# ssheybani/baby-vision-curriculum

Measured on AMD Instinct MI355X. Metric: video clips/sec (node) VideoMAE-base 16x224^2 bf16 pretraining, higher is better.
Workload: dtype bf16; 1 GPU; VideoMAE-base (ViT-B/16 encoder, 4-layer decoder), 16x224x224 clips, tubelet 2, 90% tube mask, full training step (fwd + MSE + bwd + GradScaler + SGD-Nesterov); clips_per_gpu=256, global_batch=256, parallelism=dp1, weights=random init N(0,0.02), seed 0

## Files before the change

baby-vision-curriculum_amd/csrc/attention.hip:

```cpp
#include <stdlib.h>

#include "attention.h"

namespace bvc {

#define AS3 __attribute__((address_space(3)))
#define MFMA32(a, b, c) __builtin_amdgcn_mfma_f32_32x32x16_bf16((a), (b), (c), 0, 0, 0)

template <int HD>
__device__ __forceinline__ int swz_dual(int r) {
    if constexpr (HD == 64) return (((r >> 1) & 1) << 2) | ((r >> 2) & 3);
    else return (r >> 2) & 3;
}

template <int HD>
constexpr int pan_w(int p) { return HD - 64 * p >= 64 ? 64 : HD - 64 * p; }
constexpr int img_hd(int hd) { return hd == 80 || hd == 88 ? 96 : hd; }
constexpr uint32_t kDmaZero = 0xfffffff0u;
__device__ __forceinline__ int swz_pw(int pw, int r) { return pw == 64 ? swz_dual<64>(r) : swz_dual<32>(r); }

template <int PW, int NW, int VC = PW / 8>
__device__ __forceinline__ void stage_panel(__amdgpu_buffer_rsrc_t rs, int row0, int ld, int col0, char* lds, int GB, int wave, int lane) {
    constexpr int CPR = PW / 8;
    constexpr int RPP = 64 / CPR;
#pragma unroll
    for (int jj = 0; jj < (PW / 8 + NW - 1) / NW; ++jj) {
        const int j = wave + NW * jj;
        if (NW > PW / 8 && j >= PW / 8) break;
        const int r = RPP * j + lane / CPR;
        const int c = (lane % CPR) ^ swz_dual<PW>(r);
        uint32_t off = (uint32_t)(((size_t)(row0 + r) * ld + col0 + c * 8) * 2);
        if constexpr (VC < CPR) off = c < VC ? off : kDmaZero;
        const uint32_t dst = (uint32_t)((RPP * j >> 4) * GB + ((RPP * j) & 15) * PW * 2);
        glds16(rs, off, __builtin_amdgcn_readfirstlane((uint32_t)(size_t)((AS3 char*)lds) + dst));
    }
}

template <int HD, int NW = 4, int HV = HD>
__device__ __forceinline__ void stage64(__amdgpu_buffer_rsrc_t rs, int row0, int ld, int col0, char* lds,
                                        int wave, int lane) {
    static_assert(HV == HD || (HD == 96 && HV > 64 && HV % 8 == 0), "stage64: a narrower head only on the 96 image");
    if constexpr (HD > 64) {
        stage_panel<64, NW>(rs, row0, ld, col0, lds, 16 * HD * 2, wave, lane);
        stage_panel<pan_w<HD>(1), NW, (HV - 64) / 8>(rs, row0, ld, col0 + 64, lds + 2048, 16 * HD * 2, wave, lane);
        return;
    }
    constexpr int CPR = HD / 8;
    constexpr int RPP = 64 / CPR;
#pragma unroll
    for (int jj = 0; jj < (HD / 8 + NW - 1) / NW; ++jj) {
        const int j = wave + NW * jj;
        if (NW > HD / 8 && j >= HD / 8) break;
        const int r = RPP * j + lane / CPR;
        const int c = (lane % CPR) ^ swz_dual<HD>(r);
        const uint32_t off = (uint32_t)(((size_t)(row0 + r) * ld + col0 + c * 8) * 2);
        glds16(rs, off, __builtin_amdgcn_readfirstlane((uint32_t)(size_t)((AS3 char*)lds) + (uint32_t)j * 1024u));
    }
}

template <int HD>
struct FragAddr {
    uint32_t rows[HD / 16];
    uint32_t tr[HD / 32][2];
};

template <int HD>
__device__ __forceinline__ FragAddr<HD> make_frag_addr(int lane) {
    FragAddr<HD> a;
    if constexpr (HD > 64) {
        constexpr int GB = 16 * HD * 2;
        const int r = lane & 31, h = lane >> 5, rg = r & 15;
#pragma unroll
        for (int st = 0; st < HD / 16; ++st) {
            const int pw = pan_w<HD>(st >> 2);
            a.rows[st] = (r >> 4) * GB + (st >> 2) * 2048 + rg * pw * 2 + (((2 * (st & 3) + h) ^ swz_pw(pw, rg)) << 4);
        }
        const int q = (lane >> 2) & 3, p = lane & 3;
#pragma unroll
        for (int t = 0; t < HD / 32; ++t) {
            const int pw = pan_w<HD>(t >> 1);
            const int col = 32 * (t & 1) + 16 * ((lane >> 4) & 1) + 4 * p;
            const int chunk = col >> 3, within = (col & 7) * 2;
#pragma unroll
            for (int half = 0; half < 2; ++half) {
                const int r0 = 4 * h + q + 8 * half;
                a.tr[t][half] = (t >> 1) * 2048 + r0 * pw * 2 + ((chunk ^ swz_pw(pw, r0)) << 4) + within;
            }
        }
        return a;
    }
    constexpr int RB = HD * 2;
    const int r = lane & 31, h = lane >> 5;
#pragma unroll
    for (int st = 0; st < HD / 16; ++st) a.rows[st] = r * RB + (((2 * st + h) ^ swz_dual<HD>(r)) << 4);
    const int q = (lane >> 2) & 3, p = lane & 3;
#pragma unroll
    for (int t = 0; t < HD / 32; ++t) {
        const int col = 32 * t + 16 * ((lane >> 4) & 1) + 4 * p;
        const int chunk = col >> 3, within = (col & 7) * 2;
#pragma unroll
        for (int half = 0; half < 2; ++half) {
            const int r0 = 4 * h + q + 8 * half;
            a.tr[t][half] = r0 * RB + ((chunk ^ swz_dual<HD>(r0)) << 4) + within;
        }
    }
    return a;
}

template <int IMM>
__device__ __forceinline__ bf16x8 lds_rows(const AS3 char* base, uint32_t off) {
// ... 266 lines not shown
#pragma unroll
    for (int g = 0; g < 4; ++g) {
        const f32x4 ls = *reinterpret_cast<const AS3 f32x4*>(stl + 8 * g);
#pragma unroll
        for (int e = 0; e < 4; ++e) {
            const int r = 4 * g + e;
            const float p = fast_exp2(fmaf(s[r], scale_log2, -ls[e]));
            s[r] = p;
            dp[r] = p * dp[r];
        }
    }
#endif
    if (q0 + 32 > N) {
        asm volatile("" ::: "memory");
#pragma unroll
        for (int r = 0; r < 16; ++r)
            if (q0 + acc_row(r, h) >= N) { s[r] = 0.f; dp[r] = 0.f; }
    }
    const bf16x8 p0 = acc_to_frag(s, 0), p1 = acc_to_frag(s, 1);
    const bf16x8 d0 = acc_to_frag(dp, 0), d1 = acc_to_frag(dp, 1);
#pragma unroll
    for (int t = 0; t < HD / 32; ++t) {
        dv[t] = MFMA32(lds_tr<DOFF>(lds, fa.tr[t][0], fa.tr[t][1]), p0, dv[t]);
        dk[t] = MFMA32(lds_tr<QOFF>(lds, fa.tr[t][0], fa.tr[t][1]), d0, dk[t]);
    }
#pragma unroll
    for (int t = 0; t < HD / 32; ++t) {
        dv[t] = MFMA32(lds_tr<DOFF + KS>(lds, fa.tr[t][0], fa.tr[t][1]), p1, dv[t]);
        dk[t] = MFMA32(lds_tr<QOFF + KS>(lds, fa.tr[t][0], fa.tr[t][1]), d1, dk[t]);
    }
}


template <int HD>
__global__ __launch_bounds__(256, img_hd(HD) > 96 ? 1 : 2) void attn_bwd_dkdv_kernel(const bf16_t* __restrict__ qkv, const bf16_t* __restrict__ dctx,
                                                               const float* __restrict__ lse, const float* __restrict__ delta,
                                                               bf16_t* __restrict__ dqkv, int N, int H, int D,
                                                               uint32_t qkv_bytes, uint32_t dctx_bytes, uint32_t stat_bytes,
                                                               float scale, float scale_log2, int remap) {
    constexpr bool WIN = false;
    const int q_off_ = 0, Nq_ = N;
#include "attention_dkdv_body.inc"
}
template <int HD>
__global__ __launch_bounds__(256, img_hd(HD) > 96 ? 1 : 2) void attn_bwd_dkdv_win_kernel(const bf16_t* __restrict__ qkv, const bf16_t* __restrict__ dctx,
                                                               const float* __restrict__ lse, const float* __restrict__ delta,
                                                               bf16_t* __restrict__ dqkv, int N, int H, int D,
                                                               uint32_t qkv_bytes, uint32_t dctx_bytes, uint32_t stat_bytes,
                                                               float scale, float scale_log2, int remap, int q_off_, int Nq_) {
    constexpr bool WIN = true;
#include "attention_dkdv_body.inc"
}

template <int HD, int NBT>
__global__ __launch_bounds__(320, 1) void attn_bwd_head_kernel(const bf16_t* __restrict__ qkv, const bf16_t* __restrict__ dctx,
                                                               const bf16_t* __restrict__ ctx, const float* __restrict__ lse,
                                                               bf16_t* __restrict__ dqkv, int N, int H, int D, int nheads,
                                                               uint32_t qkv_bytes, uint32_t dctx_bytes, float scale, float scale_log2) {
    static_assert(HD == 64, "whole-head backward: head_dim 64");
    extern __shared__ __attribute__((aligned(16))) char smem[];
    constexpr int IMG = 192 * HD * 2, SUB = 32 * HD * 2, KS = 16 * HD * 2;
    constexpr int QI = 0, KI = IMG, VI = 2 * IMG, OI = 3 * IMG;
    constexpr int STAT = 4 * IMG;
    constexpr int DST = STAT + 2 * 192 * 4;
    const AS3 char* lds = (const AS3 char*)smem;
    const int tid = threadIdx.x, lane = tid & 63;
    const int wave = __builtin_amdgcn_readfirstlane(tid >> 6);
    const int ld = 3 * D, h = lane >> 5;
    const int NB = NBT > 0 ? NBT : (N + 31) >> 5;
    const __amdgpu_buffer_rsrc_t rq = make_rsrc(qkv, qkv_bytes), rd = make_rsrc(dctx, dctx_bytes);
    const FragAddr<HD> fa = make_frag_addr<HD>(lane);
    const FragAddr<32> fs = make_frag_addr<32>(lane);

    auto stage_qvo = [&](int bh) __attribute__((always_inline)) {
        if (wave < 4) {
            const int b = bh / H, head = bh % H, row0 = b * N;
            for (int rb = 0; rb * 64 < N; ++rb) {
                stage64<HD>(rq, row0 + rb * 64, ld, head * HD, smem + QI + rb * 2 * SUB, wave, lane);
                stage64<HD>(rq, row0 + rb * 64, ld, 2 * D + head * HD, smem + VI + rb * 2 * SUB, wave, lane);
                stage64<HD>(rd, row0 + rb * 64, D, head * HD, smem + OI + rb * 2 * SUB, wave, lane);
            }
        }
    };
    auto stage_k = [&](int bh) __attribute__((always_inline)) {
        if (wave < 4) {
            const int b = bh / H, head = bh % H, row0 = b * N;
            for (int rb = 0; rb * 64 < N; ++rb) stage64<HD>(rq, row0 + rb * 64, ld, D + head * HD, smem + KI + rb * 2 * SUB, wave, lane);
        }
    };
    float st_lse = 0.f, st_del[5];
    auto load_stats = [&](int bh) __attribute__((always_inline)) {
        const int b = bh / H, head = bh % H;
        st_lse = (tid < N) ? lse[(size_t)bh * N + tid] : 0.f;
#pragma unroll
        for (int k = 0; k < 5; ++k) {
            const int q = (tid >> 3) + 40 * k, c = tid & 7;
            float acc = 0.f;
            if (q < N) {
                const bf16x8 dv = load8(dctx + (size_t)(b * N + q) * D + head * HD + 8 * c);
                const bf16x8 ov = load8(ctx + (size_t)(b * N + q) * D + head * HD + 8 * c);
#pragma unroll
                for (int j = 0; j < 8; ++j) acc += bf2f((bf16_t)dv[j]) * bf2f((bf16_t)ov[j]);
            }
            st_del[k] = acc;
        }
    };
    auto store_stats = [&]() __attribute__((always_inline)) {
        AS3 float* st = (AS3 float*)((AS3 char*)smem + STAT);
        if (tid < 192) st[tid] = st_lse;
#pragma unroll
        for (int k = 0; k < 5; ++k) {
            float acc = st_del[k];
            acc += __shfl_xor(acc, 1, 64);
            acc += __shfl_xor(acc, 2, 64);
            acc += __shfl_xor(acc, 4, 64);
            const int q = (tid >> 3) + 40 * k;
            if ((tid & 7) == 0 && q < 192) st[192 + q] = -acc;
        }
    };

    int bh = blockIdx.x;
    if (bh >= nheads) return;
    load_stats(bh);
    stage_qvo(bh);
    stage_k(bh);
    for (; bh < nheads; bh += gridDim.x) {
    const int b = bh / H, head = bh % H;
    const int nxt = bh + gridDim.x;
    asm volatile("s_waitcnt vmcnt(0)" ::: "memory");
    store_stats();
    __syncthreads();

    for (int kb = wave; kb < NB; kb += 5) {
        const int ki = kb * 32 + (lane & 31);
        bf16x8 kf[HD / 16], vf[HD / 16];
#pragma unroll
        for (int st = 0; st < HD / 16; ++st) {
            kf[st] = *reinterpret_cast<const AS3 bf16x8*>(lds + KI + kb * SUB + fa.rows[st]);
            vf[st] = *reinterpret_cast<const AS3 bf16x8*>(lds + VI + kb * SUB + fa.rows[st]);
        }
        f32x16 dk[HD / 32], dv[HD / 32];
#pragma unroll
        for (int t = 0; t < HD / 32; ++t) { dk[t] = zero16(); dv[t] = zero16(); }
        const bool key_ok = ki < N;
#pragma unroll
        for (int qb = 0; qb < (NBT > 0 ? NBT : NB); ++qb) {
            const AS3 char* qim = lds + QI + qb * SUB;
            const AS3 char* oim = lds + OI + qb * SUB;
            const AS3 float* stl = reinterpret_cast<const AS3 float*>(lds + STAT) + qb * 32 + 4 * h;
            f32x16 s = zero16(), dp;
#pragma unroll
            for (int g = 0; g < 4; ++g) {
                const f32x4 nd = *reinterpret_cast<const AS3 f32x4*>(stl + 192 + 8 * g);
#pragma unroll
                for (int e = 0; e < 4; ++e) dp[4 * g + e] = nd[e];
            }
#pragma unroll
            for (int stp = 0; stp < HD / 16; ++stp) {
                s = MFMA32(*reinterpret_cast<const AS3 bf16x8*>(qim + fa.rows[stp]), kf[stp], s);
                dp = MFMA32(*reinterpret_cast<const AS3 bf16x8*>(oim + fa.rows[stp]), vf[stp], dp);
            }
#pragma unroll
            for (int g = 0; g < 4; ++g) {
                const f32x4 ls = *reinterpret_cast<const AS3 f32x4*>(stl + 8 * g);
#pragma unroll
                for (int e = 0; e < 4; ++e) {
                    const int r = 4 * g + e;
                    const float pr = fast_exp2(fmaf(s[r], scale_log2, -ls[e]));
                    s[r] = pr;
                    dp[r] = pr * dp[r];
                }
            }
            if (qb * 32 + 32 > N || !__all(key_ok)) {
                asm volatile("" ::: "memory");
#pragma unroll
                for (int r = 0; r < 16; ++r)
                    if (!key_ok || qb * 32 + acc_row(r, h) >= N) { s[r] = 0.f; dp[r] = 0.f; }
            }
            const bf16x8 p0 = acc_to_frag(s, 0), p1 = acc_to_frag(s, 1);
            const bf16x8 d0 = acc_to_frag(dp, 0), d1 = acc_to_frag(dp, 1);
            {
                AS3 char* blk = (AS3 char*)smem + DST + (kb * 5 + qb) * 2048 + (lane & 31) * 64 + 8 * h;
                const int sw = swz_dual<32>(lane & 31);
                typedef __attribute__((ext_vector_type(2))) unsigned int u32x2;
                union { bf16x8 v; u32x2 u[2]; } w0, w1;
                w0.v = d0; w1.v = d1;
                *reinterpret_cast<AS3 u32x2*>(blk + ((0 ^ sw) << 4)) = w0.u[0];
                *reinterpret_cast<AS3 u32x2*>(blk + ((1 ^ sw) << 4)) = w0.u[1];
                *reinterpret_cast<AS3 u32x2*>(blk + ((2 ^ sw) << 4)) = w1.u[0];
                *reinterpret_cast<AS3 u32x2*>(blk + ((3 ^ sw) << 4)) = w1.u[1];
            }
#pragma unroll
            for (int t = 0; t < HD / 32; ++t) {
                dv[t] = MFMA32(lds_tr<0>(oim, fa.tr[t][0], fa.tr[t][1]), p0, dv[t]);
                dk[t] = MFMA32(lds_tr<0>(qim, fa.tr[t][0], fa.tr[t][1]), d0, dk[t]);
            }
#pragma unroll
            for (int t = 0; t < HD / 32; ++t) {
                dv[t] = MFMA32(lds_tr<KS>(oim, fa.tr[t][0], fa.tr[t][1]), p1, dv[t]);
                dk[t] = MFMA32(lds_tr<KS>(qim, fa.tr[t][0], fa.tr[t][1]), d1, dk[t]);
            }
        }
        if (key_ok) {
            bf16_t* krow = dqkv + (size_t)(b * N + ki) * ld + D + head * HD;
            bf16_t* vrow = krow + D;
#pragma unroll
            for (int t = 0; t < HD / 32; ++t)
#pragma unroll
                for (int g = 0; g < 4; ++g) {
                    const int d = 32 * t + 8 * g + 4 * h;
                    uint2 a = {pack2bf(dk[t][4 * g] * scale, dk[t][4 * g + 1] * scale), pack2bf(dk[t][4 * g + 2] * scale, dk[t][4 * g + 3] * scale)};
                    *reinterpret_cast<uint2*>(krow + d) = a;
                    uint2 e = {pack2bf(dv[t][4 * g], dv[t][4 * g + 1]), pack2bf(dv[t][4 * g + 2], dv[t][4 * g + 3])};
                    *reinterpret_cast<uint2*>(vrow + d) = e;
                }
        }
    }
    __syncthreads();
    if (nxt < nheads) {
        stage_qvo(nxt);
        load_stats(nxt);
    }

    for (int qb = wave; qb < NB; qb += 5) {
        const int qi = qb * 32 + (lane & 31);
        f32x16 dq[HD / 32];
#pragma unroll
        for (int t = 0; t < HD / 32; ++t) dq[t] = zero16();
#pragma unroll
        for (int kb = 0; kb < (NBT > 0 ? NBT : NB); ++kb) {
            const AS3 char* kim = lds + KI + kb * SUB;
            const AS3 char* blk = lds + DST + (kb * 5 + qb) * 2048;
            const bf16x8 b0 = lds_tr<0>(blk, fs.tr[0][0], fs.tr[0][1]);
            const bf16x8 b1 = lds_tr<1024>(blk, fs.tr[0][0], fs.tr[0][1]);
#pragma unroll
            for (int t = 0; t < HD / 32; ++t) dq[t] = MFMA32(lds_tr<0>(kim, fa.tr[t][0], fa.tr[t][1]), b0, dq[t]);
#pragma unroll
            for (int t = 0; t < HD / 32; ++t) dq[t] = MFMA32(lds_tr<KS>(kim, fa.tr[t][0], fa.tr[t][1]), b1, dq[t]);
        }
        if (qi < N) {
            bf16_t* orow = dqkv + (size_t)(b * N + qi) * ld + head * HD;
#pragma unroll
            for (int t = 0; t < HD / 32; ++t)
#pragma unroll
                for (int g = 0; g < 4; ++g) {
                    const int d = 32 * t + 8 * g + 4 * h;
                    uint2 a = {pack2bf(dq[t][4 * g] * scale, dq[t][4 * g + 1] * scale), pack2bf(dq[t][4 * g + 2] * scale, dq[t][4 * g + 3] * scale)};
                    *reinterpret_cast<uint2*>(orow + d) = a;
                }
        }
    }
    __syncthreads();
    if (nxt < nheads) stage_k(nxt);
    }
}

static int xcd_remap() {
#ifdef BVC_EXPERIMENTS
    return getenv("BVC_ATTN_PLAIN_GRID") == nullptr;
#else
    return 1;
#endif
}

static bool head_kernel_enabled() {
#ifdef BVC_EXPERIMENTS
    return getenv("BVC_ATTN_NO_HEAD_KERNEL") == nullptr;
#else
    return true;
#endif
}

template <int HD>
static int fwd_hd(const bf16_t* qkv, bf16_t* ctx, float* lse, int B, int N, int H, hipStream_t stream, float sm_scale) {
    constexpr int HI = img_hd(HD);
    const int D = H * HD;
    const size_t bytes = (size_t)B * N * 3 * D * 2;
    const float scale_log2 = (sm_scale > 0.f ? sm_scale : 1.0f / sqrtf((float)HD)) * 1.4426950408889634f;
#ifdef BVC_EXPERIMENTS
    if (getenv("BVC_ATTN_NW8") != nullptr) {
        const dim3 grid8((unsigned)(((N + 255) / 256) * B * H));
        hipLaunchKernelGGL((attn_fwd_kernel<HD, 8>), grid8, dim3(512), 4 * 64 * HI * 2, stream, qkv, ctx, lse, N, H, D, (uint32_t)bytes, scale_log2,
                           xcd_remap());
        BVC_CHECK_HIP(hipGetLastError());
        return BVC_OK;
    }
#endif
    const dim3 grid((unsigned)(((N + 127) / 128) * B * H));
    hipLaunchKernelGGL((attn_fwd_kernel<HD, 4>), grid, dim3(256), 4 * 64 * HI * 2, stream, qkv, ctx, lse, N, H, D, (uint32_t)bytes, scale_log2,
                       xcd_remap());
    BVC_CHECK_HIP(hipGetLastError());
    return BVC_OK;
}

template <int HD>
static int bwd_hd(const bf16_t* qkv, const bf16_t* ctx, const bf16_t* dctx, const float* lse, float* delta, bf16_t* dqkv, int B,
                  int N, int H, hipStream_t stream, float sm_scale, int parts) {
    constexpr int HI = img_hd(HD);
    const int D = H * HD;
    const size_t bytes = (size_t)B * N * 3 * D * 2;
    const float scale = sm_scale > 0.f ? sm_scale : 1.0f / sqrtf((float)HD), scale_log2 = scale * 1.4426950408889634f;
    const dim3 grid((unsigned)(((N + 127) / 128) * B * H));
    const int remap = xcd_remap();
    if constexpr (HD == 64) {
        if (parts == 3 && N <= 160 && head_kernel_enabled()) {
            constexpr size_t lds = 4 * 192 * HD * 2 + 2 * 192 * 4 + 25 * 2048;
            static bool attr_set = false;
            if (!attr_set) {
                BVC_CHECK_HIP(hipFuncSetAttribute(reinterpret_cast<const void*>(&attn_bwd_head_kernel<HD, 5>),
                                                  hipFuncAttributeMaxDynamicSharedMemorySize, (int)lds));
                BVC_CHECK_HIP(hipFuncSetAttribute(reinterpret_cast<const void*>(&attn_bwd_head_kernel<HD, 0>),
                                                  hipFuncAttributeMaxDynamicSharedMemorySize, (int)lds));
                attr_set = true;
            }
            static int ncu = 0;
            if (ncu == 0) {
                int dev = 0;
                hipDeviceProp_t prop;
                BVC_CHECK_HIP(hipGetDevice(&dev));
                BVC_CHECK_HIP(hipGetDeviceProperties(&prop, dev));
                ncu = prop.multiProcessorCount > 0 ? prop.multiProcessorCount : 256;
            }
            const int nheads = B * H;
            const dim3 g((unsigned)(nheads < ncu ? nheads : ncu));
            if (N > 128)
                hipLaunchKernelGGL((attn_bwd_head_kernel<HD, 5>), g, dim3(320), lds, stream, qkv, dctx, ctx, lse, dqkv, N, H, D, nheads,
                                   (uint32_t)bytes, (uint32_t)((size_t)B * N * D * 2), scale, scale_log2);
            else
                hipLaunchKernelGGL((attn_bwd_head_kernel<HD, 0>), g, dim3(320), lds, stream, qkv, dctx, ctx, lse, dqkv, N, H, D, nheads,
                                   (uint32_t)bytes, (uint32_t)((size_t)B * N * D * 2), scale, scale_log2);
            BVC_CHECK_HIP(hipGetLastError());
            return BVC_OK;
        }
    }
    if (parts & 1) {
#ifdef BVC_EXPERIMENTS
    if (HI == HD && getenv("BVC_ATTN_DQ_W") != nullptr) {
        constexpr int NB = 3;
        const dim3 gridw((unsigned)(((N + 32 * NB - 1) / (32 * NB)) * B * H));
        hipLaunchKernelGGL((attn_bwd_dq_w_kernel<HI, NB>), gridw, dim3(64), kRing * 2 * 32 * HI * 2, stream, qkv, dctx, ctx, lse, delta, dqkv, N, H, D,
                           (uint32_t)bytes, scale, scale_log2, remap);
    } else
#endif
    hipLaunchKernelGGL(attn_bwd_dq_kernel<HD>, grid, dim3(256), 4 * 64 * HI * 2, stream, qkv, dctx, ctx, lse, delta, dqkv, N, H, D,
                       (uint32_t)bytes, scale, scale_log2, remap);
    }
    if (parts & 2) {
    constexpr int lds_dkdv = 2 * (2 * 64 * HI * 2 + 512);
    if constexpr (lds_dkdv > 65536) {
        static bool attr_set = false;
        if (!attr_set) {
            BVC_CHECK_HIP(hipFuncSetAttribute(reinterpret_cast<const void*>(&attn_bwd_dkdv_kernel<HD>),
                                              hipFuncAttributeMaxDynamicSharedMemorySize, lds_dkdv));
            attr_set = true;
        }
    }
    hipLaunchKernelGGL(attn_bwd_dkdv_kernel<HD>, grid, dim3(256), lds_dkdv, stream, qkv, dctx, lse, delta, dqkv, N, H, D,
                       (uint32_t)bytes, (uint32_t)((size_t)B * N * D * 2), (uint32_t)((size_t)B * H * N * 4), scale, scale_log2, remap);
    }
    BVC_CHECK_HIP(hipGetLastError());
    return BVC_OK;
}

static bool attn_hd_ok(int hd) { return hd == 32 || hd == 64 || hd == 80 || hd == 88 || hd == 96 || hd == 128; }

int launch_attn_fwd(const bf16_t* qkv, bf16_t* ctx, float* lse, int B, int N, int H, int head_dim, hipStream_t stream, float sm_scale) {
    BVC_REQUIRE(B > 0 && N > 0 && H > 0, "attn_fwd: empty shape");
    BVC_REQUIRE(attn_hd_ok(head_dim), "attn_fwd: head_dim %d unsupported (32, 64, 80, 88, 96 or 128)", head_dim);
    BVC_REQUIRE((size_t)B * N * 3 * H * head_dim * 2 < 0xffffffffull, "attn_fwd: qkv larger than 4 GiB");
    BVC_REQUIRE(img_hd(head_dim) == head_dim || (size_t)B * N * 3 * H * head_dim * 2 < kDmaZero,
                "attn_fwd: qkv of head_dim %d must stay below 4 GiB - 16 bytes", head_dim);
    switch (head_dim) {
        case 32: return fwd_hd<32>(qkv, ctx, lse, B, N, H, stream, sm_scale);
        case 80: return fwd_hd<80>(qkv, ctx, lse, B, N, H, stream, sm_scale);
        case 88: return fwd_hd<88>(qkv, ctx, lse, B, N, H, stream, sm_scale);
        case 96: return fwd_hd<96>(qkv, ctx, lse, B, N, H, stream, sm_scale);
        case 128: return fwd_hd<128>(qkv, ctx, lse, B, N, H, stream, sm_scale);
// ... 62 lines not shown
```

baby-vision-curriculum_amd/csrc/gemm.h:

```cpp
#pragma once
#include "common.h"
#include "dropgate.h"
#include "../../include/bvc.h"

namespace bvc {

enum GemmLayout { GEMM_NT = BVC_GEMM_NT, GEMM_NN = BVC_GEMM_NN, GEMM_TN = BVC_GEMM_TN };

enum GemmEpilogue {
    EPI_F32 = BVC_EPI_F32,
    EPI_BF16 = BVC_EPI_BF16,
    EPI_GELU = BVC_EPI_GELU,
    EPI_RESID = BVC_EPI_RESID,
    EPI_POS = BVC_EPI_POS,
    EPI_E2D = BVC_EPI_E2D,
    EPI_LOSS = BVC_EPI_LOSS,
    EPI_DGELU = BVC_EPI_DGELU,
    EPI_F32_BF16 = BVC_EPI_F32_BF16,
    EPI_RELU = BVC_EPI_RELU,
    EPI_DRELU = BVC_EPI_DRELU,
    EPI_NCE = BVC_EPI_NCE,
    EPI_NCE_BWD = BVC_EPI_NCE_BWD,
    EPI_RESID_LN = BVC_EPI_RESID_LN,
    EPI_DLN = BVC_EPI_DLN,
    EPI_RESID_GATE = BVC_EPI_RESID_GATE
};

using GemmProblem = bvc_gemm_desc;

constexpr int kMaxGroup = 4;

struct Options { int gemm8 = 0; int dw_overlap = 0; int row_ln = 0; int row_stagger = 1; int deterministic = 0; int head_pad = 0; int dec_tail = 1; int dec_first = -1; };
Options& options();

float* det_scratch(size_t floats, hipStream_t stream);
size_t det_scratch_bytes();
int det_scratch_release();

struct DryRun { bool on = false; char name[160] = ""; };
DryRun& dry_run();

constexpr size_t operand_tail_bytes(size_t bf16_columns) { return 64 * bf16_columns * 2 + 1024; }
constexpr bool tn_tail_ok(int K, int ld) { return K % 64 == 0 || ((size_t)K + 63) / 64 * 64 * (size_t)ld * 2 + 1024 <= 0x100000000ull; }

int launch_gemm(const GemmProblem* probs, int nprob, GemmLayout layout, int tile_cfg, hipStream_t stream, int stages = -1);

int launch_gemm_gate(const GemmProblem& p, const Gate& gate, int tile_cfg, hipStream_t stream);

int gemm_num_tiles(const GemmProblem& p, int tile_cfg);
int gemm_pick_tile(const GemmProblem* probs, int nprob, int tile_cfg);
bool gemm_row_ln_ok(int M, int N, int K);
constexpr size_t kRowLnPartFloats = 512 * 2 * 384;

}
```

baby-vision-curriculum_amd/csrc/ops.hip:

```cpp
#include <stdarg.h>
#include <stdio.h>
#include <string.h>

#include "context.h"
#include "optim_layerwise.h"

namespace bvc {
static thread_local char g_err[1024] = "";
void set_error(const char* fmt, ...) {
    va_list ap;
    va_start(ap, fmt);
    vsnprintf(g_err, sizeof(g_err), fmt, ap);
    va_end(ap);
}
const char* last_error() { return g_err; }
}

using namespace bvc;

extern "C" {

const char* bvc_last_error(void) { return bvc::last_error(); }
const char* bvc_version(void) { return "gfx950;bvc-hip-r5"; }

int bvc_set_option(const char* name, int value) {
    BVC_REQUIRE(name != nullptr, "set_option: null name");
    if (!strcmp(name, "gemm8")) { BVC_REQUIRE(value >= -1 && value <= 1, "set_option: gemm8 takes -1 / 0 / 1"); options().gemm8 = value; }
    else if (!strcmp(name, "dw_overlap")) options().dw_overlap = value != 0;
    else if (!strcmp(name, "row_stagger")) options().row_stagger = value != 0;
    else if (!strcmp(name, "row_ln")) { BVC_REQUIRE(value >= -1 && value <= 1, "set_option: row_ln takes -1 / 0 / 1"); options().row_ln = value; }
    else if (!strcmp(name, "deterministic")) { BVC_REQUIRE(value == 0 || value == 1, "set_option: deterministic takes 0 / 1"); options().deterministic = value; }
    else if (!strcmp(name, "head_pad")) { BVC_REQUIRE(value == 0 || value == 1, "set_option: head_pad takes 0 / 1"); options().head_pad = value; }
    else if (!strcmp(name, "dec_tail")) { BVC_REQUIRE(value == 0 || value == 1, "set_option: dec_tail takes 0 / 1"); options().dec_tail = value; }
    else if (!strcmp(name, "dec_first")) { BVC_REQUIRE(value >= -1 && value <= 1, "set_option: dec_first takes -1 / 0 / 1"); options().dec_first = value; }
    else BVC_REQUIRE(false, "set_option: unknown option '%s'", name);
    return BVC_OK;
}
int bvc_get_option(const char* name) {
    if (name && !strcmp(name, "gemm8")) return options().gemm8;
    if (name && !strcmp(name, "dw_overlap")) return options().dw_overlap;
    if (name && !strcmp(name, "row_ln")) return options().row_ln;
    if (name && !strcmp(name, "row_stagger")) return options().row_stagger;
    if (name && !strcmp(name, "deterministic")) return options().deterministic;
    if (name && !strcmp(name, "head_pad")) return options().head_pad;
    if (name && !strcmp(name, "dec_tail")) return options().dec_tail;
    if (name && !strcmp(name, "dec_first")) return options().dec_first;
    bvc::set_error("get_option: unknown option '%s'", name ? name : "(null)");
    return BVC_ERR_INVALID;
}

int bvc_op_gemm(const bvc_gemm_desc* problems, int count, int layout, int tile_cfg, int stages, void* stream) {
    BVC_REQUIRE(problems, "op_gemm: null problems");
    BVC_REQUIRE(layout >= 0 && layout <= 2, "op_gemm: bad layout %d", layout);
    return launch_gemm(problems, count, (GemmLayout)layout, tile_cfg, (hipStream_t)stream, stages);
}
static int op_gate(const bvc_branch_drop* drop, int layer, int branch, int M, Gate* g) {
    BVC_REQUIRE(drop && layer >= 0 && layer < (1 << 22) && (branch == 0 || branch == 1), "gate: null description, or layer / branch out of range");
    BVC_REQUIRE(drop->hidden_p >= 0.f && drop->hidden_p < 1.f && drop->rows_per_sample >= 1, "gate: hidden_p outside [0, 1) or rows_per_sample < 1");
    const int samples = (M + drop->rows_per_sample - 1) / drop->rows_per_sample;
    *g = make_gate(drop->hidden_p, drop->seed, drop->offset,
                   drop->path_scale ? drop->path_scale + ((size_t)layer * 2 + branch) * samples : nullptr, drop->rows_per_sample, layer, branch);
    return BVC_OK;
}
int bvc_op_gemm_gate(const bvc_gemm_desc* problem, const bvc_branch_drop* drop, int layer, int branch, int tile_cfg, void* stream) {
    BVC_REQUIRE(problem, "op_gemm_gate: null problem");
    Gate g;
    TRY(op_gate(drop, layer, branch, problem->M, &g));
    return launch_gemm_gate(*problem, g, tile_cfg, (hipStream_t)stream);
}
int bvc_op_gemm_gate_kernel(const bvc_gemm_desc* problem, int tile_cfg, char* name, int name_cap) {
    BVC_REQUIRE(problem && name && name_cap > 0, "op_gemm_gate_kernel: null argument");
    DryRun& d = dry_run();
    d.on = true;
    d.name[0] = 0;
    const int rc = launch_gemm_gate(*problem, make_gate(0.f, 0, 0, nullptr, 1, 0, 0), tile_cfg, nullptr);
    d.on = false;
    if (rc == BVC_OK) snprintf(name, name_cap, "%s", d.name);
    return rc;
}
int bvc_op_dropout_mask(uint64_t seed, uint64_t offset, int layer, int branch, int M, int N, float p, uint8_t* out_dev, void* stream) {
    BVC_REQUIRE(out_dev && M >= 1 && N >= 1 && layer >= 0 && layer < (1 << 22) && (branch == 0 || branch == 1) && p >= 0.f && p < 1.f,
                "op_dropout_mask: bad argument");
    return launch_dropout_mask(make_gate(p, seed, offset, nullptr, 1, layer, branch), (size_t)M * N, out_dev, (hipStream_t)stream);
}
int bvc_dropout_mask_host(uint64_t seed, uint64_t offset, int layer, int branch, int M, int N, float p, uint8_t* out_host) {
    BVC_REQUIRE(out_host && M >= 1 && N >= 1 && layer >= 0 && layer < (1 << 22) && (branch == 0 || branch == 1) && p >= 0.f && p < 1.f,
                "dropout_mask_host: bad argument");
    dropout_mask_host(make_gate(p, seed, offset, nullptr, 1, layer, branch), (size_t)M * N, out_host);
    return BVC_OK;
}
int bvc_op_layernorm_bwd_gate(const void* dy, const float* x, const float* mean, const float* rstd, const float* gamma, float* dres,
                              int accumulate, void* dres_bf16, float* dgamma, float* dbeta, float* workspace, int M, int D,
                              const bvc_branch_drop* drop, int layer, int branch, void* stream) {
    Gate g;
    TRY(op_gate(drop, layer, branch, M, &g));
    return launch_ln_bwd((const bf16_t*)dy, x, identity_rows(), mean, rstd, gamma, dres, accumulate, (bf16_t*)dres_bf16, dgamma, dbeta,
                         workspace, M, D, (hipStream_t)stream, &g);
}
int bvc_op_gemm_kernel(const bvc_gemm_desc* problems, int count, int layout, int tile_cfg, int stages, char* name, int name_cap) {
// ... 278 lines not shown
```

baby-vision-curriculum_amd/probe.py:

```python
import ctypes

import torch

from . import _lib, _ops

PEAK_BF16_TFLOPS = 2500.0
PEAK_HBM_GBS = 8000.0


def _time(fn, iters=5, warm=2):
    for _ in range(warm):
        fn()
    e0, e1 = torch.cuda.Event(enable_timing=True), torch.cuda.Event(enable_timing=True)
    e0.record()
    for _ in range(iters):
        fn()
    e1.record()
    torch.cuda.synchronize()
    return e0.elapsed_time(e1) * 1e3 / iters


def _rb(dev, *shape):
    return torch.randn(*shape, device=dev, dtype=torch.bfloat16)

# ... 95 lines not shown
    one("dec qkv", NT, Md, 3 * Dd, Dd, "BF16", nq)
    if first:
        one("dec0 qkv (visible rows, position table)", NT, Mv + Lp, 3 * Dd, Dd, "BF16", 1)
    if fused:
        one("dec proj + LayerNorm", NT, Md, Dd, Dd, "RESID_LN", 4)
    else:
        one("dec proj", NT, Md, Dd, Dd, "RESID", 4)
    one("dec fc1+GELU", NT, Md, Id, Dd, "GELU", 4)
    if fused:
        one("dec fc2 + next LayerNorm", NT, Md, Dd, Id, "RESID_LN", 3)
        one("dec fc2", NT, Md, Dd, Id, "RESID", 1)
    else:
        one("dec fc2", NT, Md, Dd, Id, "RESID", 4)
    one("head+MSE", NT, Mm, P, Dd, "LOSS", 1)
    one("head dX", NN, Mm, Dd, P, "BF16", 1)
    one("dec dX fc2", NN, Md, Id, Dd, "DGELU", 4)
    one("dec dX fc1 + LayerNorm bwd" if fused else "dec dX fc1", NN, Md, Dd, Id, "DLN" if fused else "BF16", 4)
    one("dec dX proj", NN, Md, Dd, Dd, "BF16", 4)
    one("dec dX qkv + LayerNorm bwd" if fused else "dec dX qkv", NN, Md, Dd, 3 * Dd, "DLN" if fused else "BF16", nq)
    if first:
        one("dec0 dX qkv (visible rows)", NN, Mv, Dd, 3 * Dd, "F32" if fused else "BF16", 1)
        one("dec0 dX qkv (position sums, bf16 pair)", NN, 2 * Lp, Dd, 3 * Dd, "F32", 1)
    one("enc->dec dX", NN, Mv, D, Dd, "F32_BF16", 1)
    one("enc dX fc2", NN, Mv, I, D, "DGELU", 12)
    one("enc dX fc1", NN, Mv, D, I, "BF16", 12)
    one("enc dX proj", NN, Mv, D, D, "BF16", 12)
    one("enc dX qkv", NN, Mv, D, 3 * D, "BF16", 12)
    dw_single("head dW", P, Dd, Mm, 1)
    dw_single("enc->dec dW", Dd, D, Mv, 1)
    dw_single("patch dW", D, 1536, Mv, 1)
    dw_group("dec layer dW group", Md, Dd, Id, nq)
    if first:
        dw_group("dec0 layer dW, qkv member by position", Md, Dd, Id, 1, Kq=Mv + 2 * Lp)
    dw_group("enc layer dW group", Mv, D, I, 12)


def _attention_rows(dev, B, add):
    lib = _lib.lib()
    st = _lib.current_stream_ptr
    for label, N, H, count in (("enc", 160, 12, 12), ("dec", 1568, 6, 4)):
        Dm = 64 * H
        qkv, ctx, dctx, dqkv = _rb(dev, B * N, 3 * Dm), _rb(dev, B * N, Dm), _rb(dev, B * N, Dm), _rb(dev, B * N, 3 * Dm)
        lse = torch.empty(B * H * N, device=dev)
        delta = torch.empty(B * H * N, device=dev)
        p = lambda t: ctypes.c_void_p(t.data_ptr())
        fwd = lambda: _lib.check(lib.bvc_op_attention_fwd(p(qkv), p(ctx), p(lse), B, N, H, 64, st()), "attention_fwd")
        dq = lambda: _lib.check(lib.bvc_op_attention_bwd_part(p(qkv), p(ctx), p(dctx), p(lse), p(delta), p(dqkv), B, N, H, 64, 1, st()), "attention_bwd dq")
        dkv = lambda: _lib.check(lib.bvc_op_attention_bwd_part(p(qkv), p(ctx), p(dctx), p(lse), p(delta), p(dqkv), B, N, H, 64, 2, st()), "attention_bwd dkdv")
        unit = 2.0 * N * N * 64 * H * B
        tok = 2.0 * B * N * Dm
        add("bvc::attn_fwd_kernel<64>", f"{label} attention fwd", count, _time(fwd), 2 * unit, 4 * tok)
        if N <= 160:
            bwd = lambda: _lib.check(lib.bvc_op_attention_bwd(p(qkv), p(ctx), p(dctx), p(lse), p(delta), p(dqkv), B, N, H, 64, st()), "attention_bwd")
            add(f"bvc::attn_bwd_head_kernel<64, {5 if N > 128 else 0}>", f"{label} attention bwd (whole head: S, dP, dV, dK, dQ)", count, _time(bwd),
                5 * unit, 8 * tok)
            continue
        add("bvc::attn_bwd_dq_kernel<64>", f"{label} attention bwd dQ (S, dP, dQ)", count, _time(dq), 3 * unit, 6 * tok)
        add("bvc::attn_bwd_dkdv_kernel<64>", f"{label} attention bwd dK dV (recomputes S, dP)", count, _time(dkv), 2 * unit, 6 * tok)


def _layernorm_rows(dev, B, add):
    lib = _lib.lib()
    st = _lib.current_stream_ptr
    p = lambda t: ctypes.c_void_p(t.data_ptr())
    fused = bool(lib.bvc_op_row_ln_selected(B * 1568, 384, 1536, 6))
    for label, M, Dm, count, count_bwd in (("enc", B * 160, 768, 24, 24), ("dec", B * 1568, 384, 1 if fused else 8, 0 if fused else 8),
                                           ("final", B * 1408, 384, 1, 1)):
        x, dres = torch.randn(M, Dm, device=dev), torch.randn(M, Dm, device=dev)
        gmm, bta = torch.ones(Dm, device=dev), torch.zeros(Dm, device=dev)
        y, dy, dresb = _rb(dev, M, Dm), _rb(dev, M, Dm), _rb(dev, M, Dm)
        mean, rstd = torch.empty(M, device=dev), torch.empty(M, device=dev)
        dg, db = torch.zeros(Dm, device=dev), torch.zeros(Dm, device=dev)
        ws = torch.empty(int(lib.bvc_op_layernorm_bwd_workspace(M, Dm)), device=dev)
        fwd = lambda: _lib.check(lib.bvc_op_layernorm_fwd(p(x), 0, 0, 0, p(gmm), p(bta), p(y), p(mean), p(rstd), M, Dm, 1e-12, st()), "layernorm_fwd")
        bwd = lambda: _lib.check(lib.bvc_op_layernorm_bwd(p(dy), p(x), 0, 0, 0, p(mean), p(rstd), p(gmm), p(dres), 1, p(dresb), p(dg), p(db),
                                                          p(ws), M, Dm, st()), "layernorm_bwd")
        e = float(M) * Dm
        add("bvc::ln_fwd_kernel", f"{label} LayerNorm fwd", count, _time(fwd), 0.0, 6 * e)
        if count_bwd:
            add("bvc::ln_bwd_kernel (+ ln_param_reduce)", f"{label} LayerNorm bwd", count_bwd, _time(bwd), 0.0, 16 * e)


def step_kernels(batch, device):
    rows = {}

    def add(kernel, label, count, us, flops, nbytes):
        r = rows.setdefault(kernel, {"kernel": kernel, "launches_per_step": 0, "us_per_step": 0.0, "flops": 0.0, "bytes": 0.0, "products": []})
        r["launches_per_step"] += count
        r["us_per_step"] += count * us
        r["flops"] += count * flops
        r["bytes"] += count * nbytes
        r["products"].append({"name": label, "launches": count, "launch_us": round(us, 1),
                              "tflops": round(flops / us / 1e6, 1), "gb_per_s": round(nbytes / us / 1e3, 1)})

    with torch.no_grad():
        _gemm_rows(device, batch, add)
        _attention_rows(device, batch, add)
        _layernorm_rows(device, batch, add)
    torch.cuda.empty_cache()
    out = sorted(rows.values(), key=lambda r: -r["us_per_step"])
    total = sum(r["us_per_step"] for r in out)
    for r in out:
        us = r["us_per_step"]
        t_mfma, t_hbm = r["flops"] / (PEAK_BF16_TFLOPS * 1e6), r["bytes"] / (PEAK_HBM_GBS * 1e3)
        r["share_of_probed"] = round(us / total, 4)
        r["tflops"] = round(r["flops"] / us / 1e6, 1)
        r["gb_per_s"] = round(r["bytes"] / us / 1e3, 1)
# ... 7 lines not shown
```

Baseline: 3325 clips/s.

## Double-buffer Q/dO staging and register-prefetch K/V in whole-head attention backward

Adds a pipelined mode of the whole-head attention backward kernel, on by default. Q and dO for the next head are staged into a second LDS slot, and the next head's K/V fragments, ctx rows and LSE are loaded into registers while the current head computes. Delta is recomputed from the LDS dO copy instead of re-reading it from global memory, and the dK/dV/dQ stores are deferred until after the prefetch has landed. In exchange it uses more registers and LDS (5 images of 160 rows), which could lower occupancy or cause spills, and it needs one kernel instantiation per block count.

```diff
diff --git a/baby-vision-curriculum_amd/csrc/attention.hip b/baby-vision-curriculum_amd/csrc/attention.hip
--- a/baby-vision-curriculum_amd/csrc/attention.hip
+++ b/baby-vision-curriculum_amd/csrc/attention.hip
@@ -1,6 +1,7 @@
 #include <stdlib.h>
 
 #include "attention.h"
+#include "gemm.h"
 
 namespace bvc {
 
@@ -56,6 +57,15 @@
         const uint32_t off = (uint32_t)(((size_t)(row0 + r) * ld + col0 + c * 8) * 2);
         glds16(rs, off, __builtin_amdgcn_readfirstlane((uint32_t)(size_t)((AS3 char*)lds) + (uint32_t)j * 1024u));
     }
+}
+
+template <int HD>
+__device__ __forceinline__ void stage32(__amdgpu_buffer_rsrc_t rs, int row0, int ld, int col0, char* lds, int wave, int lane) {
+    static_assert(HD == 64, "stage32: 128-byte rows");
+    const int r = 8 * wave + (lane >> 3);
+    const int c = (lane & 7) ^ swz_dual<HD>(r);
+    const uint32_t off = (uint32_t)(((size_t)(row0 + r) * ld + col0 + c * 8) * 2);
+    glds16(rs, off, __builtin_amdgcn_readfirstlane((uint32_t)(size_t)((AS3 char*)lds) + (uint32_t)wave * 1024u));
 }
 
 template <int HD>
@@ -428,17 +438,20 @@
 #include "attention_dkdv_body.inc"
 }
 
-template <int HD, int NBT>
+template <int HD, int NBT, int MODE = 0>
 __global__ __launch_bounds__(320, 1) void attn_bwd_head_kernel(const bf16_t* __restrict__ qkv, const bf16_t* __restrict__ dctx,
                                                                const bf16_t* __restrict__ ctx, const float* __restrict__ lse,
                                                                bf16_t* __restrict__ dqkv, int N, int H, int D, int nheads,
                                                                uint32_t qkv_bytes, uint32_t dctx_bytes, float scale, float scale_log2) {
     static_assert(HD == 64, "whole-head backward: head_dim 64");
     extern __shared__ __attribute__((aligned(16))) char smem[];
-    constexpr int IMG = 192 * HD * 2, SUB = 32 * HD * 2, KS = 16 * HD * 2;
-    constexpr int QI = 0, KI = IMG, VI = 2 * IMG, OI = 3 * IMG;
-    constexpr int STAT = 4 * IMG;
-    constexpr int DST = STAT + 2 * 192 * 4;
+    constexpr bool PIPE = MODE == 1;
+    constexpr int ROWS = PIPE ? 160 : 192;
+    constexpr int IMG = ROWS * HD * 2, SUB = 32 * HD * 2, KS = 16 * HD * 2;
+    constexpr int QI = 0, KI = PIPE ? 4 * IMG : IMG, VI = 2 * IMG, OI = PIPE ? 2 * IMG : 3 * IMG;
+    constexpr int STAT = PIPE ? 5 * IMG : 4 * IMG;
+    constexpr int SST = 2 * ROWS * 4;
+    constexpr int DST = STAT + (PIPE ? 2 : 1) * SST;
     const AS3 char* lds = (const AS3 char*)smem;
     const int tid = threadIdx.x, lane = tid & 63;
     const int wave = __builtin_amdgcn_readfirstlane(tid >> 6);
@@ -481,9 +494,9 @@
             st_del[k] = acc;
         }
     };
-    auto store_stats = [&]() __attribute__((always_inline)) {
-        AS3 float* st = (AS3 float*)((AS3 char*)smem + STAT);
-        if (tid < 192) st[tid] = st_lse;
+    auto store_stats = [&](int slot) __attribute__((always_inline)) {
+        AS3 float* st = (AS3 float*)((AS3 char*)smem + STAT + slot * SST);
+        if (tid < ROWS) st[tid] = st_lse;
 #pragma unroll
         for (int k = 0; k < 5; ++k) {
             float acc = st_del[k];
@@ -491,29 +504,139 @@
             acc += __shfl_xor(acc, 2, 64);
             acc += __shfl_xor(acc, 4, 64);
             const int q = (tid >> 3) + 40 * k;
-            if ((tid & 7) == 0 && q < 192) st[192 + q] = -acc;
-        }
+            if ((tid & 7) == 0 && q < ROWS) st[ROWS + q] = -acc;
+        }
+    };
+    auto stage_img = [&](__amdgpu_buffer_rsrc_t rs, int row0, int ldx, int col0, char* img) __attribute__((always_inline)) {
+        stage64<HD>(rs, row0, ldx, col0, img, wave, lane);
+        if (N > 64) stage64<HD>(rs, row0 + 64, ldx, col0, img + 2 * SUB, wave, lane);
+        if (N > 128) stage32<HD>(rs, row0 + 128, ldx, col0, img + 4 * SUB, wave, lane);
+    };
+    auto stage_qo_slot = [&](int bh, int slot) __attribute__((always_inline)) {
+        if (wave < 4) {
+            const int b = bh / H, head = bh % H, row0 = b * N;
+            stage_img(rq, row0, ld, head * HD, smem + QI + slot * IMG);
+            stage_img(rd, row0, D, head * HD, smem + OI + slot * IMG);
+        }
+    };
+    auto stage_k_img = [&](int bh) __attribute__((always_inline)) {
+        if (wave < 4) stage_img(rq, (bh / H) * N, ld, D + (bh % H) * HD, smem + KI);
+    };
+    static_assert(!PIPE || NBT > 0, "pipelined whole-head backward: one instantiation per block count");
+    bf16x8 kfn[HD / 16], vfn[HD / 16], rov[5];
+    auto load_o = [&](int bh) __attribute__((always_inline)) {
+        const int b = bh / H, head = bh % H;
+#pragma unroll
+        for (int k = 0; k < 5; ++k) {
+            const int q = (tid >> 3) + 40 * k, c = tid & 7;
+            const bf16x8 z = {0, 0, 0, 0, 0, 0, 0, 0};
+            rov[k] = z;
+            if (q < N) rov[k] = load8(ctx + (size_t)(b * N + q) * D + head * HD + 8 * c);
+        }
+    };
+    auto load_kv = [&](int bh) __attribute__((always_inline)) {
+        const int b = bh / H, head = bh % H;
+        if (wave < NB) {
+            const bf16_t* krow = qkv + (size_t)(b * N + min(wave * 32 + (lane & 31), N - 1)) * ld + D + head * HD + 8 * h;
+#pragma unroll
+            for (int st = 0; st < HD / 16; ++st) {
+                kfn[st] = load8(krow + 16 * st);
+                vfn[st] = load8(krow + D + 16 * st);
+            }
+        }
+    };
+    auto load_next = [&](int bh) __attribute__((always_inline)) {
+        st_lse = (tid < N) ? lse[(size_t)bh * N + tid] : 0.f;
+        load_kv(bh);
+        load_o(bh);
+    };
+    auto land_next = [&]() __attribute__((always_inline)) {
+        settle(st_lse);
+#pragma unroll
+        for (int st = 0; st < HD / 16; ++st) { settle(kfn[st]); settle(vfn[st]); }
+#pragma unroll
+        for (int k = 0; k < 5; ++k) settle(rov[k]);
+        asm volatile("s_waitcnt vmcnt(0)" ::: "memory");
+    };
+    auto finish_stats = [&](int slot) __attribute__((always_inline)) {
+#pragma unroll
+        for (int k = 0; k < 5; ++k) {
+            const int q = (tid >> 3) + 40 * k, c = tid & 7;
+            bf16x8 dv = {0, 0, 0, 0, 0, 0, 0, 0};
+            if (q < N) dv = *reinterpret_cast<const AS3 bf16x8*>(lds + OI + slot * IMG + q * (HD * 2) + ((c ^ swz_dual<HD>(q)) << 4));
+            float acc = 0.f;
+#pragma unroll
+            for (int j = 0; j < 8; ++j) acc += bf2f((bf16_t)dv[j]) * bf2f((bf16_t)rov[k][j]);
+            st_del[k] = acc;
+        }
+        store_stats(slot);
     };
 
     int bh = blockIdx.x;
     if (bh >= nheads) return;
-    load_stats(bh);
-    stage_qvo(bh);
-    stage_k(bh);
+    int slot = 0;
+    if constexpr (PIPE) {
+        const bf16x8 z = {0, 0, 0, 0, 0, 0, 0, 0};
+#pragma unroll
+        for (int st = 0; st < HD / 16; ++st) { kfn[st] = z; vfn[st] = z; }
+        stage_qo_slot(bh, 0);
+        load_next(bh);
+        land_next();
+        __syncthreads();
+        finish_stats(0);
+        __syncthreads();
+    } else {
+        load_stats(bh);
+        stage_qvo(bh);
+        stage_k(bh);
+    }
     for (; bh < nheads; bh += gridDim.x) {
     const int b = bh / H, head = bh % H;
     const int nxt = bh + gridDim.x;
+    bf16x8 kfc[HD / 16], vfc[HD / 16];
+    if constexpr (PIPE) {
+#pragma unroll
+        for (int st = 0; st < HD / 16; ++st) { kfc[st] = kfn[st]; vfc[st] = vfn[st]; }
+        stage_k_img(bh);
+        if (nxt < nheads) {
+            stage_qo_slot(nxt, slot ^ 1);
+            load_next(nxt);
+        }
+    } else {
     asm volatile("s_waitcnt vmcnt(0)" ::: "memory");
-    store_stats();
+    store_stats(0);
     __syncthreads();
-
+    }
+
+    auto store_dkdv = [&](int ki, bool key_ok, const f32x16 (&dk)[HD / 32], const f32x16 (&dv)[HD / 32]) __attribute__((always_inline)) {
+        if (key_ok) {
+            bf16_t* krow = dqkv + (size_t)(b * N + ki) * ld + D + head * HD;
+            bf16_t* vrow = krow + D;
+#pragma unroll
+            for (int t = 0; t < HD / 32; ++t)
+#pragma unroll
+                for (int g = 0; g < 4; ++g) {
+                    const int d = 32 * t + 8 * g + 4 * h;
+                    uint2 a = {pack2bf(dk[t][4 * g] * scale, dk[t][4 * g + 1] * scale), pack2bf(dk[t][4 * g + 2] * scale, dk[t][4 * g + 3] * scale)};
+                    *reinterpret_cast<uint2*>(krow + d) = a;
+                    uint2 e = {pack2bf(dv[t][4 * g], dv[t][4 * g + 1]), pack2bf(dv[t][4 * g + 2], dv[t][4 * g + 3])};
+                    *reinterpret_cast<uint2*>(vrow + d) = e;
+                }
+        }
+    };
+    f32x16 pk[HD / 32], pv[HD / 32];
     for (int kb = wave; kb < NB; kb += 5) {
         const int ki = kb * 32 + (lane & 31);
         bf16x8 kf[HD / 16], vf[HD / 16];
 #pragma unroll
         for (int st = 0; st < HD / 16; ++st) {
+            if constexpr (PIPE) {
+                kf[st] = kfc[st];
+                vf[st] = vfc[st];
+            } else {
             kf[st] = *reinterpret_cast<const AS3 bf16x8*>(lds + KI + kb * SUB + fa.rows[st]);
             vf[st] = *reinterpret_cast<const AS3 bf16x8*>(lds + VI + kb * SUB + fa.rows[st]);
+            }
         }
         f32x16 dk[HD / 32], dv[HD / 32];
 #pragma unroll
@@ -521,13 +644,13 @@
         const bool key_ok = ki < N;
 #pragma unroll
         for (int qb = 0; qb < (NBT > 0 ? NBT : NB); ++qb) {
-            const AS3 char* qim = lds + QI + qb * SUB;
-            const AS3 char* oim = lds + OI + qb * SUB;
-            const AS3 float* stl = reinterpret_cast<const AS3 float*>(lds + STAT) + qb * 32 + 4 * h;
+            const AS3 char* qim = lds + QI + slot * IMG + qb * SUB;
+            const AS3 char* oim = lds + OI + slot * IMG + qb * SUB;
+            const AS3 float* stl = reinterpret_cast<const AS3 float*>(lds + STAT + slot * SST) + qb * 32 + 4 * h;
             f32x16 s = zero16(), dp;
 #pragma unroll
             for (int g = 0; g < 4; ++g) {
-                const f32x4 nd = *reinterpret_cast<const AS3 f32x4*>(stl + 192 + 8 * g);
+                const f32x4 nd = *reinterpret_cast<const AS3 f32x4*>(stl + ROWS + 8 * g);
 #pragma unroll
                 for (int e = 0; e < 4; ++e) dp[4 * g + e] = nd[e];
             }
@@ -577,6 +700,10 @@
                 dk[t] = MFMA32(lds_tr<KS>(qim, fa.tr[t][0], fa.tr[t][1]), d1, dk[t]);
             }
         }
+        if constexpr (PIPE) {
+#pragma unroll
+            for (int t = 0; t < HD / 32; ++t) { pk[t] = dk[t]; pv[t] = dv[t]; }
+        } else {
         if (key_ok) {
             bf16_t* krow = dqkv + (size_t)(b * N + ki) * ld + D + head * HD;
             bf16_t* vrow = krow + D;
@@ -591,13 +718,33 @@
                     *reinterpret_cast<uint2*>(vrow + d) = e;
                 }
         }
+        }
+    }
+    if constexpr (PIPE) {
+        land_next();
+        if (wave < NB) store_dkdv(wave * 32 + (lane & 31), wave * 32 + (lane & 31) < N, pk, pv);
     }
     __syncthreads();
+    if constexpr (MODE == 0) {
     if (nxt < nheads) {
         stage_qvo(nxt);
         load_stats(nxt);
     }
-
+    }
+
+    auto store_dq = [&](int qi, const f32x16 (&dq)[HD / 32]) __attribute__((always_inline)) {
+        if (qi < N) {
+            bf16_t* orow = dqkv + (size_t)(b * N + qi) * ld + head * HD;
+#pragma unroll
+            for (int t = 0; t < HD / 32; ++t)
+#pragma unroll
+                for (int g = 0; g < 4; ++g) {
+                    const int d = 32 * t + 8 * g + 4 * h;
+                    uint2 a = {pack2bf(dq[t][4 * g] * scale, dq[t][4 * g + 1] * scale), pack2bf(dq[t][4 * g + 2] * scale, dq[t][4 * g + 3] * scale)};
+                    *reinterpret_cast<uint2*>(orow + d) = a;
+                }
+        }
+    };
     for (int qb = wave; qb < NB; qb += 5) {
         const int qi = qb * 32 + (lane & 31);
         f32x16 dq[HD / 32];
@@ -614,6 +761,10 @@
 #pragma unroll
             for (int t = 0; t < HD / 32; ++t) dq[t] = MFMA32(lds_tr<KS>(kim, fa.tr[t][0], fa.tr[t][1]), b1, dq[t]);
         }
+        if constexpr (PIPE) {
+#pragma unroll
+            for (int t = 0; t < HD / 32; ++t) pk[t] = dq[t];
+        } else {
         if (qi < N) {
             bf16_t* orow = dqkv + (size_t)(b * N + qi) * ld + head * HD;
 #pragma unroll
@@ -625,9 +776,17 @@
                     *reinterpret_cast<uint2*>(orow + d) = a;
                 }
         }
+        }
+    }
+    if constexpr (PIPE) {
+        if (nxt < nheads) finish_stats(slot ^ 1);
+        if (wave < NB) store_dq(wave * 32 + (lane & 31), pk);
+        slot ^= 1;
     }
     __syncthreads();
+    if constexpr (MODE == 0) {
     if (nxt < nheads) stage_k(nxt);
+    }
     }
 }
 
@@ -681,12 +840,22 @@
     if constexpr (HD == 64) {
         if (parts == 3 && N <= 160 && head_kernel_enabled()) {
             constexpr size_t lds = 4 * 192 * HD * 2 + 2 * 192 * 4 + 25 * 2048;
+            constexpr size_t lds_pipe = 5 * 160 * HD * 2 + 2 * 2 * 160 * 4 + 25 * 2048;
+            static_assert(lds_pipe <= 160 * 1024, "pipelined whole-head backward: more LDS than a workgroup can have");
             static bool attr_set = false;
             if (!attr_set) {
                 BVC_CHECK_HIP(hipFuncSetAttribute(reinterpret_cast<const void*>(&attn_bwd_head_kernel<HD, 5>),
                                                   hipFuncAttributeMaxDynamicSharedMemorySize, (int)lds));
                 BVC_CHECK_HIP(hipFuncSetAttribute(reinterpret_cast<const void*>(&attn_bwd_head_kernel<HD, 0>),
                                                   hipFuncAttributeMaxDynamicSharedMemorySize, (int)lds));
+                const void* pipe[5] = {reinterpret_cast<const void*>(&attn_bwd_head_kernel<HD, 1, 1>), reinterpret_cast<const void*>(&attn_bwd_head_kernel<HD, 2, 1>),
+                                       reinterpret_cast<const void*>(&attn_bwd_head_kernel<HD, 3, 1>), reinterpret_cast<const void*>(&attn_bwd_head_kernel<HD, 4, 1>),
+                                       reinterpret_cast<const void*>(&attn_bwd_head_kernel<HD, 5, 1>)};
+                for (const void* f : pipe) BVC_CHECK_HIP(hipFuncSetAttribute(f, hipFuncAttributeMaxDynamicSharedMemorySize, (int)lds_pipe));
+#ifdef BVC_EXPERIMENTS
+                BVC_CHECK_HIP(hipFuncSetAttribute(reinterpret_cast<const void*>(&attn_bwd_head_kernel<HD, 5, 2>),
+                                                  hipFuncAttributeMaxDynamicSharedMemorySize, (int)lds));
+#endif
                 attr_set = true;
             }
             static int ncu = 0;
@@ -699,6 +868,28 @@
             }
             const int nheads = B * H;
             const dim3 g((unsigned)(nheads < ncu ? nheads : ncu));
+#ifdef BVC_EXPERIMENTS
+            if (N > 128 && getenv("BVC_ATTN_HEAD_STAGE_ONCE") != nullptr) {
+                hipLaunchKernelGGL((attn_bwd_head_kernel<HD, 5, 2>), g, dim3(320), lds, stream, qkv, dctx, ctx, lse, dqkv, N, H, D, nheads,
+                                   (uint32_t)bytes, (uint32_t)((size_t)B * N * D * 2), scale, scale_log2);
+                BVC_CHECK_HIP(hipGetLastError());
+                return BVC_OK;
+            }
+#endif
+            if (options().attn_head_pipe) {
+                const uint32_t dbytes = (uint32_t)((size_t)B * N * D * 2);
+                switch ((N + 31) >> 5) {
+#define BVC_HEAD_PIPE(NB_)                                                                                                              \
+    case NB_:                                                                                                                           \
+        hipLaunchKernelGGL((attn_bwd_head_kernel<HD, NB_, 1>), g, dim3(320), lds_pipe, stream, qkv, dctx, ctx, lse, dqkv, N, H, D, nheads, \
+                           (uint32_t)bytes, dbytes, scale, scale_log2);                                                                 \
+        break;
+                    BVC_HEAD_PIPE(1) BVC_HEAD_PIPE(2) BVC_HEAD_PIPE(3) BVC_HEAD_PIPE(4) BVC_HEAD_PIPE(5)
+#undef BVC_HEAD_PIPE
+                }
+                BVC_CHECK_HIP(hipGetLastError());
+                return BVC_OK;
+            }
             if (N > 128)
                 hipLaunchKernelGGL((attn_bwd_head_kernel<HD, 5>), g, dim3(320), lds, stream, qkv, dctx, ctx, lse, dqkv, N, H, D, nheads,
                                    (uint32_t)bytes, (uint32_t)((size_t)B * N * D * 2), scale, scale_log2);
diff --git a/baby-vision-curriculum_amd/csrc/gemm.h b/baby-vision-curriculum_amd/csrc/gemm.h
--- a/baby-vision-curriculum_amd/csrc/gemm.h
+++ b/baby-vision-curriculum_amd/csrc/gemm.h
@@ -30,7 +30,7 @@
 
 constexpr int kMaxGroup = 4;
 
-struct Options { int gemm8 = 0; int dw_overlap = 0; int row_ln = 0; int row_stagger = 1; int deterministic = 0; int head_pad = 0; int dec_tail = 1; int dec_first = -1; };
+struct Options { int gemm8 = 0; int dw_overlap = 0; int row_ln = 0; int row_stagger = 1; int deterministic = 0; int head_pad = 0; int dec_tail = 1; int dec_first = -1; int attn_head_pipe = 1; };
 Options& options();
 
 float* det_scratch(size_t floats, hipStream_t stream);
diff --git a/baby-vision-curriculum_amd/csrc/ops.hip b/baby-vision-curriculum_amd/csrc/ops.hip
--- a/baby-vision-curriculum_amd/csrc/ops.hip
+++ b/baby-vision-curriculum_amd/csrc/ops.hip
@@ -33,6 +33,7 @@
     else if (!strcmp(name, "head_pad")) { BVC_REQUIRE(value == 0 || value == 1, "set_option: head_pad takes 0 / 1"); options().head_pad = value; }
     else if (!strcmp(name, "dec_tail")) { BVC_REQUIRE(value == 0 || value == 1, "set_option: dec_tail takes 0 / 1"); options().dec_tail = value; }
     else if (!strcmp(name, "dec_first")) { BVC_REQUIRE(value >= -1 && value <= 1, "set_option: dec_first takes -1 / 0 / 1"); options().dec_first = value; }
+    else if (!strcmp(name, "attn_head_pipe")) { BVC_REQUIRE(value == 0 || value == 1, "set_option: attn_head_pipe takes 0 / 1"); options().attn_head_pipe = value; }
     else BVC_REQUIRE(false, "set_option: unknown option '%s'", name);
     return BVC_OK;
 }
@@ -45,6 +46,7 @@
     if (name && !strcmp(name, "head_pad")) return options().head_pad;
     if (name && !strcmp(name, "dec_tail")) return options().dec_tail;
     if (name && !strcmp(name, "dec_first")) return options().dec_first;
+    if (name && !strcmp(name, "attn_head_pipe")) return options().attn_head_pipe;
     bvc::set_error("get_option: unknown option '%s'", name ? name : "(null)");
     return BVC_ERR_INVALID;
 }
diff --git a/baby-vision-curriculum_amd/probe.py b/baby-vision-curriculum_amd/probe.py
--- a/baby-vision-curriculum_amd/probe.py
+++ b/baby-vision-curriculum_amd/probe.py
@@ -171,7 +171,8 @@
         add("bvc::attn_fwd_kernel<64>", f"{label} attention fwd", count, _time(fwd), 2 * unit, 4 * tok)
         if N <= 160:
             bwd = lambda: _lib.check(lib.bvc_op_attention_bwd(p(qkv), p(ctx), p(dctx), p(lse), p(delta), p(dqkv), B, N, H, 64, st()), "attention_bwd")
-            add(f"bvc::attn_bwd_head_kernel<64, {5 if N > 128 else 0}>", f"{label} attention bwd (whole head: S, dP, dV, dK, dQ)", count, _time(bwd),
+            inst = f"{(N + 31) // 32}, 1" if lib.bvc_get_option(b"attn_head_pipe") == 1 else f"{5 if N > 128 else 0}, 0"
+            add(f"bvc::attn_bwd_head_kernel<64, {inst}>", f"{label} attention bwd (whole head: S, dP, dV, dK, dQ)", count, _time(bwd),
                 5 * unit, 8 * tok)
             continue
         add("bvc::attn_bwd_dq_kernel<64>", f"{label} attention bwd dQ (S, dP, dQ)", count, _time(dq), 3 * unit, 6 * tok)
```

Result: no change. 3347 clips/s (median of 6 runs) (+0.7%).
